# lifeiteng/vall-e

Measured on NVIDIA H100. Metric: audio tokens/sec (AR+NAR d=1024/12L), higher is better.
Workload: dtype bf16

## Files before the change

valle_b200/csrc/gemm_wgmma.cu:

```cuda
#include <cuda.h>
#include <stdlib.h>

#include "common.cuh"
#include "kernels.cuh"
#include "sm90_ptx.cuh"

namespace vb {

namespace tc {

constexpr int BM = 128, BN = 128;
constexpr int kThreads = 384;
constexpr int kStages = 6;
constexpr int kABytes = BM * BK * 2;
constexpr int kBBytes = BN * BK * 2;
constexpr int kStageBytes = kABytes + kBBytes;
constexpr int kSmemBytes = kStages * kStageBytes + 1024  + 256 ;
static_assert(kSmemBytes <= 227 * 1024, "shared memory of one CTA");

template <int kEpi, typename TC>
__global__ void __launch_bounds__(kThreads, 1)
gemm_wgmma_kernel(const __grid_constant__ CUtensorMap tmap_a, const __grid_constant__ CUtensorMap tmap_b,
                  const float *__restrict__ bias, TC *__restrict__ C, int64_t ldc, int M, int K) {
  extern __shared__ uint8_t smem_raw[];
  uint8_t *tiles = reinterpret_cast<uint8_t *>((reinterpret_cast<uintptr_t>(smem_raw) + 1023) & ~(uintptr_t)1023);
  uint64_t *bars = reinterpret_cast<uint64_t *>(tiles + kStages * kStageBytes);
  uint64_t *full_bar = bars;
  uint64_t *empty_bar = bars + kStages;

  const int wg = threadIdx.x >> 7, t = threadIdx.x & 127;
  const int n_blk = blockIdx.x, m_blk = blockIdx.y;
  const int num_kb = K / BK;

  if (threadIdx.x == 0) {
    prefetch_tmap(&tmap_a);
    prefetch_tmap(&tmap_b);
    for (int i = 0; i < kStages; ++i) {
      mbar_init(&full_bar[i], 1);
      mbar_init(&empty_bar[i], 8);
    }
    asm volatile("fence.mbarrier_init.release.cluster;" ::: "memory");
  }
  __syncthreads();

  if (wg == 0) {
    if (t == 0) {
      int stage = 0;
      uint32_t phase = 0;
      for (int kb = 0; kb < num_kb; ++kb) {
        mbar_wait(&empty_bar[stage], phase ^ 1);
        uint8_t *a_dst = tiles + stage * kStageBytes;
        mbar_expect_tx(&full_bar[stage], kStageBytes);
        tma_load_2d(&tmap_a, &full_bar[stage], a_dst, kb * BK, m_blk * BM);
        tma_load_2d(&tmap_b, &full_bar[stage], a_dst + kABytes, kb * BK, n_blk * BN);
        if (++stage == kStages) {
          stage = 0;
          phase ^= 1;
        }
      }
    }
    return;
  }

  const int half = wg - 1;
  float acc[BN / 2];
  int stage = 0, prev = -1;
  uint32_t phase = 0;
  for (int kb = 0; kb < num_kb; ++kb) {
    mbar_wait(&full_bar[stage], phase);
    const uint32_t a_addr = smem_u32(tiles + stage * kStageBytes) + half * (64 * 128);
    const uint32_t b_addr = smem_u32(tiles + stage * kStageBytes) + kABytes;
    const uint64_t adesc = make_smem_desc(a_addr), bdesc = make_smem_desc(b_addr);
    wgmma_fence();
#pragma unroll
    for (int k = 0; k < BK / WGMMA_K; ++k) wgmma_m64n128k16(acc, adesc + (uint64_t)(k * 2), bdesc + (uint64_t)(k * 2), (kb | k) != 0);
    wgmma_commit();
    wgmma_wait<1>();
    if (prev >= 0 && (t & 31) == 0) mbar_arrive(&empty_bar[prev]);
    prev = stage;
    if (++stage == kStages) {
      stage = 0;
      phase ^= 1;
    }
  }
  wgmma_wait<0>();
  wgmma_fence_regs(acc);

  const int n0 = n_blk * BN;
#pragma unroll
  for (int i = 0; i < BN / 2; i += 2) {
    const int row = m_blk * BM + half * 64 + wg_row(t, i);
    const int col = n0 + wg_col(t, i);
    if (row >= M) continue;
    float v0 = acc[i], v1 = acc[i + 1];
    if (bias) {
      v0 += __ldg(bias + col);
      v1 += __ldg(bias + col + 1);
    }
    if constexpr (kEpi == VB_EPI_RELU) {
      v0 = fmaxf(v0, 0.f);
      v1 = fmaxf(v1, 0.f);
    }
    TC *dst = C + (int64_t)row * ldc + col;
    if constexpr (sizeof(TC) == 4) {
      float2 *d2 = reinterpret_cast<float2 *>(dst);
      if constexpr (kEpi == VB_EPI_RESIDUAL) {
        const float2 o = *d2;
        v0 = o.x + v0;
        v1 = o.y + v1;
      }
      *d2 = make_float2(v0, v1);
    } else {
      *reinterpret_cast<__nv_bfloat162 *>(dst) = __floats2bfloat162_rn(v0, v1);
    }
  }
}

template <int kEpi, typename TC>
static int launch_t(const CUtensorMap &ta, const CUtensorMap &tb, const float *bias, TC *C, int64_t ldc, int M,
                    int N, int K, cudaStream_t s) {
  auto kern = gemm_wgmma_kernel<kEpi, TC>;
  static PerDeviceOnce once;
  if (once.first()) VB_CUDA(cudaFuncSetAttribute(kern, cudaFuncAttributeMaxDynamicSharedMemorySize, kSmemBytes));
  const dim3 grid(N / BN, (M + BM - 1) / BM);
  kern<<<grid, kThreads, kSmemBytes, s>>>(ta, tb, bias, C, ldc, M, K);
  VB_LAUNCH_CHECK();
  return VB_OK;
}

}

bool wgmma_gemm_supported(int64_t M, int N, int K, int64_t lda, int64_t ldc) {
  return M >= 1 && (M + tc::BM - 1) / tc::BM <= 65535 && N % tc::BN == 0 && K % tc::BK == 0 && K > 0 &&
         lda % 8 == 0 && ldc % 8 == 0 && getenv("VB_DISABLE_WGMMA") == nullptr;
}

int launch_gemm_wgmma(const bf16 *A, int64_t lda, const bf16 *W, const float *bias, void *C, int c_dtype,
                      int64_t ldc, int64_t M, int N, int K, int epi, cudaStream_t s) {
  VB_CHECK_ARG((reinterpret_cast<uintptr_t>(A) & 15) == 0 && (reinterpret_cast<uintptr_t>(W) & 15) == 0 &&
                   (reinterpret_cast<uintptr_t>(C) & 15) == 0,
               "wgmma gemm: operands must be 16-byte aligned");
  CUtensorMap ta, tb;
  VB_TRY(tc::make_tmap(&ta, A, M, K, lda, tc::BM));
  VB_TRY(tc::make_tmap(&tb, W, N, K, K, tc::BN));
  const int m = (int)M;
  if (epi == VB_EPI_RESIDUAL) return tc::launch_t<VB_EPI_RESIDUAL, float>(ta, tb, bias, (float *)C, ldc, m, N, K, s);
  if (epi == VB_EPI_RELU) {
    if (c_dtype == VB_BF16) return tc::launch_t<VB_EPI_RELU, bf16>(ta, tb, bias, (bf16 *)C, ldc, m, N, K, s);
    return tc::launch_t<VB_EPI_RELU, float>(ta, tb, bias, (float *)C, ldc, m, N, K, s);
  }
  if (c_dtype == VB_BF16) return tc::launch_t<VB_EPI_NONE, bf16>(ta, tb, bias, (bf16 *)C, ldc, m, N, K, s);
  return tc::launch_t<VB_EPI_NONE, float>(ta, tb, bias, (float *)C, ldc, m, N, K, s);
}

}
```

valle_b200/csrc/sm90_ptx.cuh:

```cuda
#pragma once
#include <cuda.h>

#include <mutex>

#include "common.cuh"

namespace vb {
namespace tc {

constexpr int BK = 64;
constexpr int WGMMA_K = 16;

__device__ __forceinline__ uint32_t smem_u32(const void *p) {
  return static_cast<uint32_t>(__cvta_generic_to_shared(p));
}
__device__ __forceinline__ void mbar_init(uint64_t *bar, uint32_t count) {
  asm volatile("mbarrier.init.shared::cta.b64 [%0], %1;" ::"r"(smem_u32(bar)), "r"(count));
}
__device__ __forceinline__ void mbar_expect_tx(uint64_t *bar, uint32_t bytes) {
  asm volatile("mbarrier.arrive.expect_tx.shared::cta.b64 _, [%0], %1;" ::"r"(smem_u32(bar)), "r"(bytes)
               : "memory");
}
__device__ __forceinline__ void mbar_arrive(uint64_t *bar) {
  asm volatile("mbarrier.arrive.shared::cta.b64 _, [%0];" ::"r"(smem_u32(bar)) : "memory");
}
__device__ __forceinline__ uint32_t mbar_try_wait(uint64_t *bar, uint32_t parity) {
  uint32_t ok;
  asm volatile(
      "{\n"
      ".reg .pred p;\n"
      "mbarrier.try_wait.parity.shared::cta.b64 p, [%1], %2;\n"
      "selp.u32 %0, 1, 0, p;\n"
      "}\n"
      : "=r"(ok)
      : "r"(smem_u32(bar)), "r"(parity)
      : "memory");
  return ok;
}
__device__ __forceinline__ void mbar_wait(uint64_t *bar, uint32_t parity) {
  while (!mbar_try_wait(bar, parity)) {
  }
}
__device__ __forceinline__ void tma_load_2d(const CUtensorMap *map, uint64_t *bar, void *dst, int c0, int c1) {
  asm volatile(
      "cp.async.bulk.tensor.2d.shared::cluster.global.tile.mbarrier::complete_tx::bytes [%0], [%1, {%3, %4}], [%2];"
      ::"r"(smem_u32(dst)), "l"(map), "r"(smem_u32(bar)), "r"(c0), "r"(c1)
      : "memory");
}
__device__ __forceinline__ void prefetch_tmap(const CUtensorMap *map) {
  asm volatile("prefetch.tensormap [%0];" ::"l"(map) : "memory");
}
__device__ __forceinline__ void wgmma_fence() { asm volatile("wgmma.fence.sync.aligned;" ::: "memory"); }
__device__ __forceinline__ void wgmma_commit() { asm volatile("wgmma.commit_group.sync.aligned;" ::: "memory"); }
template <int N> __device__ __forceinline__ void wgmma_wait() {
  asm volatile("wgmma.wait_group.sync.aligned %0;" ::"n"(N) : "memory");
}
template <int R> __device__ __forceinline__ void wgmma_fence_regs(float (&d)[R]) {
#pragma unroll
  for (int i = 0; i < R; ++i) asm volatile("" : "+f"(d[i])::"memory");
}
__device__ __forceinline__ uint64_t make_smem_desc(uint32_t smem_addr) {
  uint64_t d = 0;
  d |= (uint64_t)((smem_addr & 0x3FFFF) >> 4);
  d |= (uint64_t)1 << 16;
  d |= (uint64_t)(1024 >> 4) << 32;
  d |= (uint64_t)1 << 62;
  return d;
}
__device__ __forceinline__ int wg_row(int t, int i) { return ((t >> 5) << 4) + ((t & 31) >> 2) + (((i >> 1) & 1) << 3); }
__device__ __forceinline__ int wg_col(int t, int i) { return ((i >> 2) << 3) + ((t & 3) << 1) + (i & 1); }

__device__ __forceinline__ void wgmma_m64n64k16(float (&d)[32], uint64_t adesc, uint64_t bdesc, uint32_t accumulate) {
  asm volatile(
      "{\n"
      ".reg .pred p;\n"
      "setp.ne.b32 p, %34, 0;\n"
      "wgmma.mma_async.sync.aligned.m64n64k16.f32.bf16.bf16 "
      "{%0, %1, %2, %3, %4, %5, %6, %7, %8, %9, %10, %11, %12, %13, %14, %15, %16, %17, %18, %19, %20, %21, %22, %23, %24, %25, %26, %27, %28, %29, %30, %31}, "
      "%32, %33, p, 1, 1, 0, 0;\n"
      "}\n"
      : "+f"(d[0]), "+f"(d[1]), "+f"(d[2]), "+f"(d[3]), "+f"(d[4]), "+f"(d[5]), "+f"(d[6]), "+f"(d[7]), "+f"(d[8]), "+f"(d[9]), "+f"(d[10]), "+f"(d[11]), "+f"(d[12]), "+f"(d[13]), "+f"(d[14]), "+f"(d[15]), "+f"(d[16]), "+f"(d[17]), "+f"(d[18]), "+f"(d[19]), "+f"(d[20]), "+f"(d[21]), "+f"(d[22]), "+f"(d[23]), "+f"(d[24]), "+f"(d[25]), "+f"(d[26]), "+f"(d[27]), "+f"(d[28]), "+f"(d[29]), "+f"(d[30]), "+f"(d[31])
      : "l"(adesc), "l"(bdesc), "r"(accumulate));
}

__device__ __forceinline__ void wgmma_m64n128k16(float (&d)[64], uint64_t adesc, uint64_t bdesc, uint32_t accumulate) {
  asm volatile(
      "{\n"
      ".reg .pred p;\n"
      "setp.ne.b32 p, %66, 0;\n"
      "wgmma.mma_async.sync.aligned.m64n128k16.f32.bf16.bf16 "
      "{%0, %1, %2, %3, %4, %5, %6, %7, %8, %9, %10, %11, %12, %13, %14, %15, %16, %17, %18, %19, %20, %21, %22, %23, %24, %25, %26, %27, %28, %29, %30, %31, %32, %33, %34, %35, %36, %37, %38, %39, %40, %41, %42, %43, %44, %45, %46, %47, %48, %49, %50, %51, %52, %53, %54, %55, %56, %57, %58, %59, %60, %61, %62, %63}, "
      "%64, %65, p, 1, 1, 0, 0;\n"
      "}\n"
      : "+f"(d[0]), "+f"(d[1]), "+f"(d[2]), "+f"(d[3]), "+f"(d[4]), "+f"(d[5]), "+f"(d[6]), "+f"(d[7]), "+f"(d[8]), "+f"(d[9]), "+f"(d[10]), "+f"(d[11]), "+f"(d[12]), "+f"(d[13]), "+f"(d[14]), "+f"(d[15]), "+f"(d[16]), "+f"(d[17]), "+f"(d[18]), "+f"(d[19]), "+f"(d[20]), "+f"(d[21]), "+f"(d[22]), "+f"(d[23]), "+f"(d[24]), "+f"(d[25]), "+f"(d[26]), "+f"(d[27]), "+f"(d[28]), "+f"(d[29]), "+f"(d[30]), "+f"(d[31]), "+f"(d[32]), "+f"(d[33]), "+f"(d[34]), "+f"(d[35]), "+f"(d[36]), "+f"(d[37]), "+f"(d[38]), "+f"(d[39]), "+f"(d[40]), "+f"(d[41]), "+f"(d[42]), "+f"(d[43]), "+f"(d[44]), "+f"(d[45]), "+f"(d[46]), "+f"(d[47]), "+f"(d[48]), "+f"(d[49]), "+f"(d[50]), "+f"(d[51]), "+f"(d[52]), "+f"(d[53]), "+f"(d[54]), "+f"(d[55]), "+f"(d[56]), "+f"(d[57]), "+f"(d[58]), "+f"(d[59]), "+f"(d[60]), "+f"(d[61]), "+f"(d[62]), "+f"(d[63])
      : "l"(adesc), "l"(bdesc), "r"(accumulate));
}

__device__ __forceinline__ void wgmma_m64n64k16_rs_tb(float (&d)[32], const uint32_t (&a)[4], uint64_t bdesc) {
  asm volatile(
      "{\n"
      ".reg .pred p;\n"
      "setp.ne.b32 p, %37, 0;\n"
      "wgmma.mma_async.sync.aligned.m64n64k16.f32.bf16.bf16 "
      "{%0, %1, %2, %3, %4, %5, %6, %7, %8, %9, %10, %11, %12, %13, %14, %15, %16, %17, %18, %19, %20, %21, %22, %23, %24, %25, %26, %27, %28, %29, %30, %31}, "
      "{%32, %33, %34, %35}, %36, p, 1, 1, 1;\n"
      "}\n"
      : "+f"(d[0]), "+f"(d[1]), "+f"(d[2]), "+f"(d[3]), "+f"(d[4]), "+f"(d[5]), "+f"(d[6]), "+f"(d[7]), "+f"(d[8]), "+f"(d[9]), "+f"(d[10]), "+f"(d[11]), "+f"(d[12]), "+f"(d[13]), "+f"(d[14]), "+f"(d[15]), "+f"(d[16]), "+f"(d[17]), "+f"(d[18]), "+f"(d[19]), "+f"(d[20]), "+f"(d[21]), "+f"(d[22]), "+f"(d[23]), "+f"(d[24]), "+f"(d[25]), "+f"(d[26]), "+f"(d[27]), "+f"(d[28]), "+f"(d[29]), "+f"(d[30]), "+f"(d[31])
      : "r"(a[0]), "r"(a[1]), "r"(a[2]), "r"(a[3]), "l"(bdesc), "r"(1));
}

typedef CUresult (*EncodeTiledFn)(CUtensorMap *, CUtensorMapDataType, cuuint32_t, void *, const cuuint64_t *,
                                  const cuuint64_t *, const cuuint32_t *, const cuuint32_t *,
                                  CUtensorMapInterleave, CUtensorMapSwizzle, CUtensorMapL2promotion,
                                  CUtensorMapFloatOOBfill);

inline EncodeTiledFn get_encode() {
  static EncodeTiledFn fn = nullptr;
  static std::once_flag once;
  std::call_once(once, [] {
    void *p = nullptr;
    cudaDriverEntryPointQueryResult q;
    if (cudaGetDriverEntryPoint("cuTensorMapEncodeTiled", &p, cudaEnableDefault, &q) == cudaSuccess &&
        q == cudaDriverEntryPointSuccess)
      fn = reinterpret_cast<EncodeTiledFn>(p);
  });
  return fn;
}

inline int make_tmap_f32_dense(CUtensorMap *map, const void *ptr, int64_t rows, int64_t cols, int64_t ld, int box_rows,
                               int box_cols) {
  EncodeTiledFn enc = get_encode();
  if (!enc) {
    set_error("tensor map: cuTensorMapEncodeTiled entry point unavailable");
    return VB_ERR_CUDA;
  }
  cuuint64_t dims[2] = {(cuuint64_t)cols, (cuuint64_t)rows};
  cuuint64_t strides[1] = {(cuuint64_t)ld * 4};
  cuuint32_t box[2] = {(cuuint32_t)box_cols, (cuuint32_t)box_rows};
  cuuint32_t estr[2] = {1, 1};
  CUresult r = enc(map, CU_TENSOR_MAP_DATA_TYPE_FLOAT32, 2, const_cast<void *>(ptr), dims, strides, box, estr,
                   CU_TENSOR_MAP_INTERLEAVE_NONE, CU_TENSOR_MAP_SWIZZLE_NONE, CU_TENSOR_MAP_L2_PROMOTION_L2_256B,
                   CU_TENSOR_MAP_FLOAT_OOB_FILL_NONE);
  if (r != CUDA_SUCCESS) {
    set_error("tensor map: cuTensorMapEncodeTiled (fp32 dense) failed (%d) rows=%lld cols=%lld ld=%lld", (int)r,
              (long long)rows, (long long)cols, (long long)ld);
    return VB_ERR_CUDA;
  }
  return VB_OK;
}
inline int make_tmap(CUtensorMap *map, const void *ptr, int64_t rows, int K, int64_t ld, int box_rows) {
  EncodeTiledFn enc = get_encode();
  if (!enc) {
    set_error("wgmma gemm: cuTensorMapEncodeTiled entry point unavailable");
    return VB_ERR_CUDA;
  }
  cuuint64_t dims[2] = {(cuuint64_t)K, (cuuint64_t)rows};
  cuuint64_t strides[1] = {(cuuint64_t)ld * 2};
  cuuint32_t box[2] = {(cuuint32_t)BK, (cuuint32_t)box_rows};
  cuuint32_t estr[2] = {1, 1};
  CUresult r = enc(map, CU_TENSOR_MAP_DATA_TYPE_BFLOAT16, 2, const_cast<void *>(ptr), dims, strides, box, estr,
                   CU_TENSOR_MAP_INTERLEAVE_NONE, CU_TENSOR_MAP_SWIZZLE_128B, CU_TENSOR_MAP_L2_PROMOTION_L2_256B,
                   CU_TENSOR_MAP_FLOAT_OOB_FILL_NONE);
  if (r != CUDA_SUCCESS) {
    set_error("wgmma gemm: cuTensorMapEncodeTiled failed (%d) rows=%lld K=%d ld=%lld", (int)r, (long long)rows, K,
              (long long)ld);
    return VB_ERR_CUDA;
  }
  return VB_OK;
}

}
}
```

Measured before the change: 296,600.

## Make WGMMA GEMM persistent with 128x256 tiles and TMA-store epilogue

Rewrites the Hopper GEMM as a persistent kernel sized to the SM count that loops over tiles. The tile grows to 128x256 using m64n256 WGMMA, with fewer pipeline stages and setmaxnreg to move registers from the producer to the consumers. The epilogue now stages results in swizzled shared memory and writes them with TMA bulk stores. For the residual case, the old tile is TMA-loaded through the operand ring instead of read directly from global memory. This aims to raise compute per loaded byte, cut launch and tail overhead, and coalesce output writes, at the cost of register pressure, a shallower pipeline, and tile padding when N is not a multiple of 256.

```diff
diff --git a/valle_b200/csrc/gemm_wgmma.cu b/valle_b200/csrc/gemm_wgmma.cu
--- a/valle_b200/csrc/gemm_wgmma.cu
+++ b/valle_b200/csrc/gemm_wgmma.cu
@@ -9,32 +9,46 @@
 
 namespace tc {
 
-constexpr int BM = 128, BN = 128;
+constexpr int BM = 128, BN = 256;
 constexpr int kThreads = 384;
-constexpr int kStages = 6;
+constexpr int kStages = 4;
 constexpr int kABytes = BM * BK * 2;
 constexpr int kBBytes = BN * BK * 2;
 constexpr int kStageBytes = kABytes + kBBytes;
-constexpr int kSmemBytes = kStages * kStageBytes + 1024  + 256 ;
+constexpr int kStgBytes = 64 * 128;
+constexpr int kXBoxBytes = BM * 128;
+constexpr int kXBoxes = BN / 32;
+constexpr int kXPerStage = kStageBytes / kXBoxBytes;
+constexpr int kXStages = (kXBoxes + kXPerStage - 1) / kXPerStage;
+constexpr int kSmemBytes = kStages * kStageBytes + 4 * kStgBytes + 1024  + 256 ;
 static_assert(kSmemBytes <= 227 * 1024, "shared memory of one CTA");
+static_assert(kXStages <= kStages, "x of a tile fits the ring");
 
 template <int kEpi, typename TC>
 __global__ void __launch_bounds__(kThreads, 1)
 gemm_wgmma_kernel(const __grid_constant__ CUtensorMap tmap_a, const __grid_constant__ CUtensorMap tmap_b,
-                  const float *__restrict__ bias, TC *__restrict__ C, int64_t ldc, int M, int K) {
+                  const __grid_constant__ CUtensorMap tmap_c, const __grid_constant__ CUtensorMap tmap_x,
+                  const float *__restrict__ bias, int M, int N, int K) {
+  constexpr bool kRes = kEpi == VB_EPI_RESIDUAL;
+  constexpr int SUBN = 128 / (int)sizeof(TC);
+  static_assert(!kRes || SUBN == 32, "residual sub-tiles are the x boxes' columns");
   extern __shared__ uint8_t smem_raw[];
   uint8_t *tiles = reinterpret_cast<uint8_t *>((reinterpret_cast<uintptr_t>(smem_raw) + 1023) & ~(uintptr_t)1023);
-  uint64_t *bars = reinterpret_cast<uint64_t *>(tiles + kStages * kStageBytes);
+  uint8_t *stg = tiles + kStages * kStageBytes;
+  uint64_t *bars = reinterpret_cast<uint64_t *>(stg + 4 * kStgBytes);
   uint64_t *full_bar = bars;
   uint64_t *empty_bar = bars + kStages;
 
   const int wg = threadIdx.x >> 7, t = threadIdx.x & 127;
-  const int n_blk = blockIdx.x, m_blk = blockIdx.y;
+  const int n_tiles = (N + BN - 1) / BN;
+  const int num_tiles = ((M + BM - 1) / BM) * n_tiles;
   const int num_kb = K / BK;
 
   if (threadIdx.x == 0) {
     prefetch_tmap(&tmap_a);
     prefetch_tmap(&tmap_b);
+    prefetch_tmap(&tmap_c);
+    if constexpr (kRes) prefetch_tmap(&tmap_x);
     for (int i = 0; i < kStages; ++i) {
       mbar_init(&full_bar[i], 1);
       mbar_init(&empty_bar[i], 8);
@@ -43,87 +57,141 @@
   }
   __syncthreads();
 
-  if (wg == 0) {
-    if (t == 0) {
-      int stage = 0;
-      uint32_t phase = 0;
-      for (int kb = 0; kb < num_kb; ++kb) {
-        mbar_wait(&empty_bar[stage], phase ^ 1);
-        uint8_t *a_dst = tiles + stage * kStageBytes;
-        mbar_expect_tx(&full_bar[stage], kStageBytes);
-        tma_load_2d(&tmap_a, &full_bar[stage], a_dst, kb * BK, m_blk * BM);
-        tma_load_2d(&tmap_b, &full_bar[stage], a_dst + kABytes, kb * BK, n_blk * BN);
-        if (++stage == kStages) {
-          stage = 0;
-          phase ^= 1;
-        }
-      }
-    }
-    return;
-  }
-
-  const int half = wg - 1;
-  float acc[BN / 2];
-  int stage = 0, prev = -1;
+  int stage = 0;
   uint32_t phase = 0;
-  for (int kb = 0; kb < num_kb; ++kb) {
-    mbar_wait(&full_bar[stage], phase);
-    const uint32_t a_addr = smem_u32(tiles + stage * kStageBytes) + half * (64 * 128);
-    const uint32_t b_addr = smem_u32(tiles + stage * kStageBytes) + kABytes;
-    const uint64_t adesc = make_smem_desc(a_addr), bdesc = make_smem_desc(b_addr);
-    wgmma_fence();
-#pragma unroll
-    for (int k = 0; k < BK / WGMMA_K; ++k) wgmma_m64n128k16(acc, adesc + (uint64_t)(k * 2), bdesc + (uint64_t)(k * 2), (kb | k) != 0);
-    wgmma_commit();
-    wgmma_wait<1>();
-    if (prev >= 0 && (t & 31) == 0) mbar_arrive(&empty_bar[prev]);
-    prev = stage;
+  auto advance = [&] {
     if (++stage == kStages) {
       stage = 0;
       phase ^= 1;
     }
-  }
-  wgmma_wait<0>();
-  wgmma_fence_regs(acc);
-
-  const int n0 = n_blk * BN;
+  };
+
+  if (wg == 0) {
+    setmaxnreg_dec<40>();
+    if (t == 0) {
+      for (int tile = blockIdx.x; tile < num_tiles; tile += gridDim.x) {
+        const int m0 = (tile / n_tiles) * BM, n0 = (tile % n_tiles) * BN;
+        for (int kb = 0; kb < num_kb; ++kb) {
+          mbar_wait(&empty_bar[stage], phase ^ 1);
+          uint8_t *a_dst = tiles + stage * kStageBytes;
+          mbar_expect_tx(&full_bar[stage], kStageBytes);
+          tma_load_2d(&tmap_a, &full_bar[stage], a_dst, kb * BK, m0);
+          tma_load_2d(&tmap_b, &full_bar[stage], a_dst + kABytes, kb * BK, n0);
+          advance();
+        }
+        if constexpr (kRes) {
+          for (int q = 0; q < kXStages; ++q) {
+            mbar_wait(&empty_bar[stage], phase ^ 1);
+            int nbox = 0;
+            for (int j = 0; j < kXPerStage; ++j) {
+              const int b = q * kXPerStage + j;
+              nbox += (b < kXBoxes && n0 + 32 * b < N);
+            }
+            mbar_expect_tx(&full_bar[stage], nbox * kXBoxBytes);
+            for (int j = 0; j < nbox; ++j)
+              tma_load_2d(&tmap_x, &full_bar[stage], tiles + stage * kStageBytes + j * kXBoxBytes,
+                          n0 + 32 * (q * kXPerStage + j), m0);
+            advance();
+          }
+        }
+      }
+    }
+    return;
+  }
+
+  setmaxnreg_inc<232>();
+  const int half = wg - 1;
+  uint8_t *my_stg = stg + half * 2 * kStgBytes;
+  int sbuf = 0;
+  float acc[BN / 2];
+  for (int tile = blockIdx.x; tile < num_tiles; tile += gridDim.x) {
+    const int m0 = (tile / n_tiles) * BM, n0 = (tile % n_tiles) * BN;
+    int prev = 0;
+    for (int kb = 0; kb < num_kb; ++kb) {
+      mbar_wait(&full_bar[stage], phase);
+      const uint32_t a_addr = smem_u32(tiles + stage * kStageBytes) + half * (64 * 128);
+      const uint32_t b_addr = smem_u32(tiles + stage * kStageBytes) + kABytes;
+      const uint64_t adesc = make_smem_desc(a_addr), bdesc = make_smem_desc(b_addr);
+      wgmma_fence();
 #pragma unroll
-  for (int i = 0; i < BN / 2; i += 2) {
-    const int row = m_blk * BM + half * 64 + wg_row(t, i);
-    const int col = n0 + wg_col(t, i);
-    if (row >= M) continue;
-    float v0 = acc[i], v1 = acc[i + 1];
-    if (bias) {
-      v0 += __ldg(bias + col);
-      v1 += __ldg(bias + col + 1);
-    }
-    if constexpr (kEpi == VB_EPI_RELU) {
-      v0 = fmaxf(v0, 0.f);
-      v1 = fmaxf(v1, 0.f);
-    }
-    TC *dst = C + (int64_t)row * ldc + col;
-    if constexpr (sizeof(TC) == 4) {
-      float2 *d2 = reinterpret_cast<float2 *>(dst);
-      if constexpr (kEpi == VB_EPI_RESIDUAL) {
-        const float2 o = *d2;
-        v0 = o.x + v0;
-        v1 = o.y + v1;
-      }
-      *d2 = make_float2(v0, v1);
-    } else {
-      *reinterpret_cast<__nv_bfloat162 *>(dst) = __floats2bfloat162_rn(v0, v1);
-    }
-  }
+      for (int k = 0; k < BK / WGMMA_K; ++k)
+        wgmma_m64n256k16(acc, adesc + (uint64_t)(k * 2), bdesc + (uint64_t)(k * 2), (kb | k) != 0);
+      wgmma_commit();
+      wgmma_wait<1>();
+      if (kb > 0 && (t & 31) == 0) mbar_arrive(&empty_bar[prev]);
+      prev = stage;
+      advance();
+    }
+    wgmma_wait<0>();
+    wgmma_fence_regs(acc);
+    if ((t & 31) == 0) mbar_arrive(&empty_bar[prev]);
+
+    const int row0 = m0 + half * 64;
+#pragma unroll
+    for (int sub = 0; sub < BN / SUBN; ++sub) {
+      const int c0 = n0 + sub * SUBN;
+      if constexpr (kRes) {
+        if (sub % kXPerStage == 0) mbar_wait(&full_bar[stage], phase);
+      }
+      if (c0 < N && row0 < M) {
+        uint8_t *buf = my_stg + sbuf * kStgBytes;
+        if (t == 0) bulk_wait_read<1>();
+        named_bar_sync(1 + half, 128);
+#pragma unroll
+        for (int i = sub * (SUBN / 2); i < (sub + 1) * (SUBN / 2); i += 2) {
+          const int r = wg_row(t, i), cc = wg_col(t, i) - sub * SUBN;
+          const int byte = cc * (int)sizeof(TC);
+          const int off = r * 128 + ((((byte >> 4) ^ r) & 7) << 4) + (byte & 15);
+          float v0 = acc[i], v1 = acc[i + 1];
+          if (bias) {
+            v0 += __ldg(bias + c0 + cc);
+            v1 += __ldg(bias + c0 + cc + 1);
+          }
+          if constexpr (kEpi == VB_EPI_RELU) {
+            v0 = fmaxf(v0, 0.f);
+            v1 = fmaxf(v1, 0.f);
+          }
+          if constexpr (sizeof(TC) == 4) {
+            if constexpr (kRes) {
+              const float2 o = *reinterpret_cast<const float2 *>(
+                  tiles + stage * kStageBytes + (sub % kXPerStage) * kXBoxBytes + half * (64 * 128) + off);
+              v0 = o.x + v0;
+              v1 = o.y + v1;
+            }
+            *reinterpret_cast<float2 *>(buf + off) = make_float2(v0, v1);
+          } else {
+            *reinterpret_cast<__nv_bfloat162 *>(buf + off) = __floats2bfloat162_rn(v0, v1);
+          }
+        }
+        fence_proxy_async_smem();
+        named_bar_sync(1 + half, 128);
+        if (t == 0) {
+          tma_store_2d(&tmap_c, buf, c0, row0);
+          bulk_commit();
+        }
+        sbuf ^= 1;
+      }
+      if constexpr (kRes) {
+        if (sub % kXPerStage == kXPerStage - 1 || sub == BN / SUBN - 1) {
+          __syncwarp();
+          if ((t & 31) == 0) mbar_arrive(&empty_bar[stage]);
+          advance();
+        }
+      }
+    }
+  }
+  if (t == 0) bulk_wait<0>();
 }
 
 template <int kEpi, typename TC>
-static int launch_t(const CUtensorMap &ta, const CUtensorMap &tb, const float *bias, TC *C, int64_t ldc, int M,
-                    int N, int K, cudaStream_t s) {
+static int launch_t(const CUtensorMap &ta, const CUtensorMap &tb, const CUtensorMap &tc_, const CUtensorMap &tx,
+                    const float *bias, int M, int N, int K, cudaStream_t s) {
   auto kern = gemm_wgmma_kernel<kEpi, TC>;
   static PerDeviceOnce once;
   if (once.first()) VB_CUDA(cudaFuncSetAttribute(kern, cudaFuncAttributeMaxDynamicSharedMemorySize, kSmemBytes));
-  const dim3 grid(N / BN, (M + BM - 1) / BM);
-  kern<<<grid, kThreads, kSmemBytes, s>>>(ta, tb, bias, C, ldc, M, K);
+  const int tiles = ((M + BM - 1) / BM) * ((N + BN - 1) / BN);
+  const int grid = tiles < sm_count() ? tiles : sm_count();
+  kern<<<grid, kThreads, kSmemBytes, s>>>(ta, tb, tc_, tx, bias, M, N, K);
   VB_LAUNCH_CHECK();
   return VB_OK;
 }
@@ -131,7 +199,7 @@
 }
 
 bool wgmma_gemm_supported(int64_t M, int N, int K, int64_t lda, int64_t ldc) {
-  return M >= 1 && (M + tc::BM - 1) / tc::BM <= 65535 && N % tc::BN == 0 && K % tc::BK == 0 && K > 0 &&
+  return M >= 1 && (M + tc::BM - 1) / tc::BM <= 65535 && N % 128 == 0 && K % tc::BK == 0 && K > 0 &&
          lda % 8 == 0 && ldc % 8 == 0 && getenv("VB_DISABLE_WGMMA") == nullptr;
 }
 
@@ -140,17 +208,21 @@
   VB_CHECK_ARG((reinterpret_cast<uintptr_t>(A) & 15) == 0 && (reinterpret_cast<uintptr_t>(W) & 15) == 0 &&
                    (reinterpret_cast<uintptr_t>(C) & 15) == 0,
                "wgmma gemm: operands must be 16-byte aligned");
-  CUtensorMap ta, tb;
+  const bool f32 = epi == VB_EPI_RESIDUAL || c_dtype != VB_BF16;
+  CUtensorMap ta, tb, tcm, tx;
   VB_TRY(tc::make_tmap(&ta, A, M, K, lda, tc::BM));
   VB_TRY(tc::make_tmap(&tb, W, N, K, K, tc::BN));
+  VB_TRY(tc::make_tmap_swz128(&tcm, C, f32, M, N, ldc, 64));
+  tx = tcm;
+  if (epi == VB_EPI_RESIDUAL) VB_TRY(tc::make_tmap_swz128(&tx, C, true, M, N, ldc, tc::BM));
   const int m = (int)M;
-  if (epi == VB_EPI_RESIDUAL) return tc::launch_t<VB_EPI_RESIDUAL, float>(ta, tb, bias, (float *)C, ldc, m, N, K, s);
+  if (epi == VB_EPI_RESIDUAL) return tc::launch_t<VB_EPI_RESIDUAL, float>(ta, tb, tcm, tx, bias, m, N, K, s);
   if (epi == VB_EPI_RELU) {
-    if (c_dtype == VB_BF16) return tc::launch_t<VB_EPI_RELU, bf16>(ta, tb, bias, (bf16 *)C, ldc, m, N, K, s);
-    return tc::launch_t<VB_EPI_RELU, float>(ta, tb, bias, (float *)C, ldc, m, N, K, s);
-  }
-  if (c_dtype == VB_BF16) return tc::launch_t<VB_EPI_NONE, bf16>(ta, tb, bias, (bf16 *)C, ldc, m, N, K, s);
-  return tc::launch_t<VB_EPI_NONE, float>(ta, tb, bias, (float *)C, ldc, m, N, K, s);
-}
-
-}
+    if (c_dtype == VB_BF16) return tc::launch_t<VB_EPI_RELU, bf16>(ta, tb, tcm, tx, bias, m, N, K, s);
+    return tc::launch_t<VB_EPI_RELU, float>(ta, tb, tcm, tx, bias, m, N, K, s);
+  }
+  if (c_dtype == VB_BF16) return tc::launch_t<VB_EPI_NONE, bf16>(ta, tb, tcm, tx, bias, m, N, K, s);
+  return tc::launch_t<VB_EPI_NONE, float>(ta, tb, tcm, tx, bias, m, N, K, s);
+}
+
+}
diff --git a/valle_b200/csrc/sm90_ptx.cuh b/valle_b200/csrc/sm90_ptx.cuh
--- a/valle_b200/csrc/sm90_ptx.cuh
+++ b/valle_b200/csrc/sm90_ptx.cuh
@@ -49,6 +49,30 @@
 }
 __device__ __forceinline__ void prefetch_tmap(const CUtensorMap *map) {
   asm volatile("prefetch.tensormap [%0];" ::"l"(map) : "memory");
+}
+__device__ __forceinline__ void tma_store_2d(const CUtensorMap *map, const void *src, int c0, int c1) {
+  asm volatile("cp.async.bulk.tensor.2d.global.shared::cta.bulk_group [%0, {%2, %3}], [%1];" ::"l"(map),
+               "r"(smem_u32(src)), "r"(c0), "r"(c1)
+               : "memory");
+}
+__device__ __forceinline__ void bulk_commit() { asm volatile("cp.async.bulk.commit_group;" ::: "memory"); }
+template <int N> __device__ __forceinline__ void bulk_wait_read() {
+  asm volatile("cp.async.bulk.wait_group.read %0;" ::"n"(N) : "memory");
+}
+template <int N> __device__ __forceinline__ void bulk_wait() {
+  asm volatile("cp.async.bulk.wait_group %0;" ::"n"(N) : "memory");
+}
+__device__ __forceinline__ void fence_proxy_async_smem() {
+  asm volatile("fence.proxy.async.shared::cta;" ::: "memory");
+}
+__device__ __forceinline__ void named_bar_sync(int id, int threads) {
+  asm volatile("bar.sync %0, %1;" ::"r"(id), "r"(threads) : "memory");
+}
+template <int R> __device__ __forceinline__ void setmaxnreg_inc() {
+  asm volatile("setmaxnreg.inc.sync.aligned.u32 %0;" ::"n"(R));
+}
+template <int R> __device__ __forceinline__ void setmaxnreg_dec() {
+  asm volatile("setmaxnreg.dec.sync.aligned.u32 %0;" ::"n"(R));
 }
 __device__ __forceinline__ void wgmma_fence() { asm volatile("wgmma.fence.sync.aligned;" ::: "memory"); }
 __device__ __forceinline__ void wgmma_commit() { asm volatile("wgmma.commit_group.sync.aligned;" ::: "memory"); }
@@ -83,16 +107,16 @@
       : "l"(adesc), "l"(bdesc), "r"(accumulate));
 }
 
-__device__ __forceinline__ void wgmma_m64n128k16(float (&d)[64], uint64_t adesc, uint64_t bdesc, uint32_t accumulate) {
-  asm volatile(
-      "{\n"
-      ".reg .pred p;\n"
-      "setp.ne.b32 p, %66, 0;\n"
-      "wgmma.mma_async.sync.aligned.m64n128k16.f32.bf16.bf16 "
-      "{%0, %1, %2, %3, %4, %5, %6, %7, %8, %9, %10, %11, %12, %13, %14, %15, %16, %17, %18, %19, %20, %21, %22, %23, %24, %25, %26, %27, %28, %29, %30, %31, %32, %33, %34, %35, %36, %37, %38, %39, %40, %41, %42, %43, %44, %45, %46, %47, %48, %49, %50, %51, %52, %53, %54, %55, %56, %57, %58, %59, %60, %61, %62, %63}, "
-      "%64, %65, p, 1, 1, 0, 0;\n"
-      "}\n"
-      : "+f"(d[0]), "+f"(d[1]), "+f"(d[2]), "+f"(d[3]), "+f"(d[4]), "+f"(d[5]), "+f"(d[6]), "+f"(d[7]), "+f"(d[8]), "+f"(d[9]), "+f"(d[10]), "+f"(d[11]), "+f"(d[12]), "+f"(d[13]), "+f"(d[14]), "+f"(d[15]), "+f"(d[16]), "+f"(d[17]), "+f"(d[18]), "+f"(d[19]), "+f"(d[20]), "+f"(d[21]), "+f"(d[22]), "+f"(d[23]), "+f"(d[24]), "+f"(d[25]), "+f"(d[26]), "+f"(d[27]), "+f"(d[28]), "+f"(d[29]), "+f"(d[30]), "+f"(d[31]), "+f"(d[32]), "+f"(d[33]), "+f"(d[34]), "+f"(d[35]), "+f"(d[36]), "+f"(d[37]), "+f"(d[38]), "+f"(d[39]), "+f"(d[40]), "+f"(d[41]), "+f"(d[42]), "+f"(d[43]), "+f"(d[44]), "+f"(d[45]), "+f"(d[46]), "+f"(d[47]), "+f"(d[48]), "+f"(d[49]), "+f"(d[50]), "+f"(d[51]), "+f"(d[52]), "+f"(d[53]), "+f"(d[54]), "+f"(d[55]), "+f"(d[56]), "+f"(d[57]), "+f"(d[58]), "+f"(d[59]), "+f"(d[60]), "+f"(d[61]), "+f"(d[62]), "+f"(d[63])
+__device__ __forceinline__ void wgmma_m64n256k16(float (&d)[128], uint64_t adesc, uint64_t bdesc, uint32_t accumulate) {
+  asm volatile(
+      "{\n"
+      ".reg .pred p;\n"
+      "setp.ne.b32 p, %130, 0;\n"
+      "wgmma.mma_async.sync.aligned.m64n256k16.f32.bf16.bf16 "
+      "{%0, %1, %2, %3, %4, %5, %6, %7, %8, %9, %10, %11, %12, %13, %14, %15, %16, %17, %18, %19, %20, %21, %22, %23, %24, %25, %26, %27, %28, %29, %30, %31, %32, %33, %34, %35, %36, %37, %38, %39, %40, %41, %42, %43, %44, %45, %46, %47, %48, %49, %50, %51, %52, %53, %54, %55, %56, %57, %58, %59, %60, %61, %62, %63, %64, %65, %66, %67, %68, %69, %70, %71, %72, %73, %74, %75, %76, %77, %78, %79, %80, %81, %82, %83, %84, %85, %86, %87, %88, %89, %90, %91, %92, %93, %94, %95, %96, %97, %98, %99, %100, %101, %102, %103, %104, %105, %106, %107, %108, %109, %110, %111, %112, %113, %114, %115, %116, %117, %118, %119, %120, %121, %122, %123, %124, %125, %126, %127}, "
+      "%128, %129, p, 1, 1, 0, 0;\n"
+      "}\n"
+      : "+f"(d[0]), "+f"(d[1]), "+f"(d[2]), "+f"(d[3]), "+f"(d[4]), "+f"(d[5]), "+f"(d[6]), "+f"(d[7]), "+f"(d[8]), "+f"(d[9]), "+f"(d[10]), "+f"(d[11]), "+f"(d[12]), "+f"(d[13]), "+f"(d[14]), "+f"(d[15]), "+f"(d[16]), "+f"(d[17]), "+f"(d[18]), "+f"(d[19]), "+f"(d[20]), "+f"(d[21]), "+f"(d[22]), "+f"(d[23]), "+f"(d[24]), "+f"(d[25]), "+f"(d[26]), "+f"(d[27]), "+f"(d[28]), "+f"(d[29]), "+f"(d[30]), "+f"(d[31]), "+f"(d[32]), "+f"(d[33]), "+f"(d[34]), "+f"(d[35]), "+f"(d[36]), "+f"(d[37]), "+f"(d[38]), "+f"(d[39]), "+f"(d[40]), "+f"(d[41]), "+f"(d[42]), "+f"(d[43]), "+f"(d[44]), "+f"(d[45]), "+f"(d[46]), "+f"(d[47]), "+f"(d[48]), "+f"(d[49]), "+f"(d[50]), "+f"(d[51]), "+f"(d[52]), "+f"(d[53]), "+f"(d[54]), "+f"(d[55]), "+f"(d[56]), "+f"(d[57]), "+f"(d[58]), "+f"(d[59]), "+f"(d[60]), "+f"(d[61]), "+f"(d[62]), "+f"(d[63]), "+f"(d[64]), "+f"(d[65]), "+f"(d[66]), "+f"(d[67]), "+f"(d[68]), "+f"(d[69]), "+f"(d[70]), "+f"(d[71]), "+f"(d[72]), "+f"(d[73]), "+f"(d[74]), "+f"(d[75]), "+f"(d[76]), "+f"(d[77]), "+f"(d[78]), "+f"(d[79]), "+f"(d[80]), "+f"(d[81]), "+f"(d[82]), "+f"(d[83]), "+f"(d[84]), "+f"(d[85]), "+f"(d[86]), "+f"(d[87]), "+f"(d[88]), "+f"(d[89]), "+f"(d[90]), "+f"(d[91]), "+f"(d[92]), "+f"(d[93]), "+f"(d[94]), "+f"(d[95]), "+f"(d[96]), "+f"(d[97]), "+f"(d[98]), "+f"(d[99]), "+f"(d[100]), "+f"(d[101]), "+f"(d[102]), "+f"(d[103]), "+f"(d[104]), "+f"(d[105]), "+f"(d[106]), "+f"(d[107]), "+f"(d[108]), "+f"(d[109]), "+f"(d[110]), "+f"(d[111]), "+f"(d[112]), "+f"(d[113]), "+f"(d[114]), "+f"(d[115]), "+f"(d[116]), "+f"(d[117]), "+f"(d[118]), "+f"(d[119]), "+f"(d[120]), "+f"(d[121]), "+f"(d[122]), "+f"(d[123]), "+f"(d[124]), "+f"(d[125]), "+f"(d[126]), "+f"(d[127])
       : "l"(adesc), "l"(bdesc), "r"(accumulate));
 }
 
@@ -148,6 +172,28 @@
   }
   return VB_OK;
 }
+inline int make_tmap_swz128(CUtensorMap *map, const void *ptr, bool f32, int64_t rows, int64_t cols, int64_t ld,
+                            int box_rows) {
+  EncodeTiledFn enc = get_encode();
+  if (!enc) {
+    set_error("tensor map: cuTensorMapEncodeTiled entry point unavailable");
+    return VB_ERR_CUDA;
+  }
+  const int esz = f32 ? 4 : 2;
+  cuuint64_t dims[2] = {(cuuint64_t)cols, (cuuint64_t)rows};
+  cuuint64_t strides[1] = {(cuuint64_t)(ld * esz)};
+  cuuint32_t box[2] = {(cuuint32_t)(128 / esz), (cuuint32_t)box_rows};
+  cuuint32_t estr[2] = {1, 1};
+  CUresult r = enc(map, f32 ? CU_TENSOR_MAP_DATA_TYPE_FLOAT32 : CU_TENSOR_MAP_DATA_TYPE_BFLOAT16, 2,
+                   const_cast<void *>(ptr), dims, strides, box, estr, CU_TENSOR_MAP_INTERLEAVE_NONE,
+                   CU_TENSOR_MAP_SWIZZLE_128B, CU_TENSOR_MAP_L2_PROMOTION_L2_256B, CU_TENSOR_MAP_FLOAT_OOB_FILL_NONE);
+  if (r != CUDA_SUCCESS) {
+    set_error("tensor map: cuTensorMapEncodeTiled (swizzled output) failed (%d) rows=%lld cols=%lld ld=%lld", (int)r,
+              (long long)rows, (long long)cols, (long long)ld);
+    return VB_ERR_CUDA;
+  }
+  return VB_OK;
+}
 inline int make_tmap(CUtensorMap *map, const void *ptr, int64_t rows, int K, int64_t ld, int box_rows) {
   EncodeTiledFn enc = get_encode();
   if (!enc) {
```

Result: faster. 331,100 (median of 6 runs) (+11.6%).
